# TengdaHan/TemporalAlignNet

Hardware: AMD Instinct MI355X
Metric: video-seq/sec (len=64, E6D6) at 1/2/4/8 MI355X; HTM-Align ROC-AUC parity (higher is better)
Workload: dtype bf16; 1 GPU; E6D6 len=64 bf16 stage-1 (init: multi-positive NCE only) train step (fwd+loss+bwd+AdamW), synthetic HTM-370K-shaped features, N~U[4,16] sentences/video; global_batch=128, per_gpu_batch=128, seq_len=64, parallelism=dp1

## Files before the change

include/tan_hip.h:

```cpp
#ifndef TAN_HIP_H
#define TAN_HIP_H

#ifdef __cplusplus
extern "C" {
#endif

#define TAN_F32 0
#define TAN_BF16 1
#define TAN_ERR_BAD_ARG (-1)

#define TAN_ACT_NONE 0
#define TAN_ACT_QUICKGELU 1
#define TAN_ACT_QUICKGELU_GRAD 2
#define TAN_ACT_RELU 3

int tan_version(void);
int tan_abi_sizeof(int which);

#define TAN_PROF_GEMM_BF16 0
#define TAN_PROF_GEMM_F32 4
#define TAN_PROF_ATTN_FWD 8
#define TAN_PROF_ATTN_BWD 9
#define TAN_PROF_SIMNCE 10
#define TAN_PROF_PANEL 11
// ... 173 lines not shown
    long unit_begin, unit_end;
} tan_adamw_images_desc;
int tan_adamw_step_images(const tan_adamw_images_desc* d, void* stream);
int tan_ema_update(float* target, const float* online, long n, float m, void* target_bf16, void* stream);

int tan_clip_chunk(void);
int tan_clip_sumsq(const float* g, const int* chunk_table, const int* seg_table, int c0, int c1, int s0, int s1, long n,
                   float* partials, void* stream);
int tan_clip_apply(float* g, const int* chunk_table, const int* seg_table, int c0, int c1, int s0, int s1, long n,
                   const float* partials, float clip, float grad_scale, float* norms, void* stream);

typedef struct tan_layer_params {
    const void *w_qkv, *w_out, *w_fc, *w_proj;
    const float *b_qkv, *b_out, *b_fc, *b_proj;
    const float *ln1_g, *ln1_b, *ln2_g, *ln2_b;
    float *g_w_qkv, *g_w_out, *g_w_fc, *g_w_proj;
    float *g_b_qkv, *g_b_out, *g_b_fc, *g_b_proj;
    float *g_ln1_g, *g_ln1_b, *g_ln2_g, *g_ln2_b;
    const void *wt_qkv, *wt_out, *wt_fc, *wt_proj;
    const void *wp_qkv, *wp_out, *wp_fc, *wp_proj;
    const void *wtp_qkv, *wtp_out, *wtp_fc, *wtp_proj;
} tan_layer_params;

typedef struct tan_layer_bufs {
    void *xn1, *qkv, *attn_o, *x_mid, *xn2, *h_pre, *h_act, *x_out;
    float *mean1, *rstd1, *mean2, *rstd2;
    float* lse;
} tan_layer_bufs;

typedef struct tan_encoder_desc {
    int dtype, B, L, C, H, layers;
    const unsigned char* key_padding_mask;
    const void* x0;
    const tan_layer_params* params;
    const tan_layer_bufs* bufs;
    const float *post_g, *post_b;
    float *g_post_g, *g_post_b;
    void* post_out;
    float *post_mean, *post_rstd;
    void *scr_dx, *scr_dx2, *scr_do, *scr_dxn;
    void* scr_dh;
    void* scr_dqkv;
    float* ln_ws;
    float* dw_ws;
    long dw_ws_floats;
    const void* const* d_stage;
    void* d_x0;
    void* const* layer_done;
    int no_save;
    int xn1_ready;
    void* dw_stream; int dw_tail;
    void *scr2_dx, *scr2_dx2, *scr2_dh, *scr2_dqkv;
    float* split_part;
} tan_encoder_desc;
int tan_encoder_fwd(const tan_encoder_desc* e, void* stream);
int tan_encoder_bwd(const tan_encoder_desc* e, void* stream);

int tan_linear_wgrad(const void* dy, const void* x, float* gw, long M, int N, int K, float* ws, long ws_floats, int dtype,
                     void* stream);
int tan_gemm_atb(int n, const void* const* A, const void* const* B, void* const* C, const int* lda, const int* M, const int* N, long K,
                 int out_dtype, int accumulate, int split, void* stream);
int tan_linear_wgrad_group(int n, const void* const* dy, const void* const* x, float* const* gw, const int* N, const int* K,
                           long M, float* ws, long ws_floats, int dtype, void* stream);

typedef struct tan_pack_entry { long src_off, dst_off; int N, K, TN, TK; } tan_pack_entry;
int tan_panel_waves(void);
int tan_pack_weights(const void* src, void* dst, const tan_pack_entry* table, int n, int max_tiles, void* stream);

typedef struct tan_mlp_desc {
    long rows; int C, FF;
    const void* x_mid;
    const float *ln_g, *ln_b;
    const void *pw_fc, *pw_proj;
    const float *b_fc, *b_proj;
    void* xn2; float *mean2, *rstd2;
    void *h_pre, *h_act;
    void* x_out;
    const float *nln_g, *nln_b;
    void* xn_next; float *nmean, *nrstd;
    float eps;
    int variant;
    const void* attn_o; const void* pw_out; const float* b_out; const void* x_in;
} tan_mlp_desc;
int tan_mlp_fwd(const tan_mlp_desc* d, void* stream);

typedef struct tan_mlp_bwd_desc {
    long rows; int C, FF;
    const void* dx;
    const void* h_pre;
    const void* x_mid;
    const float *mean2, *rstd2, *ln_g;
    const void *pwt_proj, *pwt_fc;
    void* dh;
    void* dx2;
    float *g_b_fc, *g_ln_g, *g_ln_b, *g_b_out;
    const void *ln1_dxn, *ln1_x, *ln1_res;
    const float *ln1_mean, *ln1_rstd, *ln1_g;
    float *g_ln1_g, *g_ln1_b, *g_dx_colsum;
    void* dx_out;
    const void* pwt_out;
    void* d_o;
    const void* dqkv;
    const void* pwt_in;
    const void* dstage;
} tan_mlp_bwd_desc;
int tan_mlp_bwd(const tan_mlp_bwd_desc* d, void* stream);
// ... 137 lines not shown
```

temporalalignnet_amd/_lib.py:

```python
from __future__ import annotations

import ctypes as C
import os
import re

HERE = os.path.dirname(os.path.abspath(__file__))
LIB_PATH = os.environ.get("TAN_HIP_LIB") or os.path.join(HERE, "libtan_hip.so")
HEADER = os.path.join(HERE, "..", "include", "tan_hip.h")

TAN_F32, TAN_BF16 = 0, 1
ACT_NONE, ACT_QUICKGELU, ACT_QUICKGELU_GRAD, ACT_RELU = 0, 1, 2, 3


class TanHipError(RuntimeError):
    pass


class GemmDesc(C.Structure):
    _fields_ = [
        ("dtype", C.c_int), ("out_dtype", C.c_int),
        ("M", C.c_int), ("N", C.c_int), ("K", C.c_int),
        ("a_kc", C.c_int), ("b_kc", C.c_int),
        ("A", C.c_void_p), ("lda", C.c_long),
        ("B", C.c_void_p), ("ldb", C.c_long),
# ... 157 lines not shown
        ("pwt_out", C.c_void_p), ("d_o", C.c_void_p),
        ("dqkv", C.c_void_p), ("pwt_in", C.c_void_p), ("dstage", C.c_void_p),
    ]


class EmbedDesc(C.Structure):
    _fields_ = [
        ("a", C.c_void_p), ("a_dtype", C.c_int), ("rows", C.c_long), ("K", C.c_int), ("T", C.c_int), ("C", C.c_int),
        ("pw", C.c_void_p), ("ln_g", C.c_void_p), ("ln_b", C.c_void_p),
        ("a_bf16", C.c_void_p), ("proj", C.c_void_p), ("mean", C.c_void_p), ("rstd", C.c_void_p),
        ("out", C.c_void_p * 2), ("out_grp_rows", C.c_long * 2), ("out_off", C.c_long * 2), ("pos", C.c_void_p * 2),
        ("ln1_g", C.c_void_p * 2), ("ln1_b", C.c_void_p * 2), ("xn1", C.c_void_p * 2), ("mean1", C.c_void_p * 2), ("rstd1", C.c_void_p * 2),
        ("pad_src", C.c_void_p), ("pad_dst", C.c_void_p), ("pad_grp_rows", C.c_long), ("pad_off", C.c_long),
    ]


class EmbedBwdDesc(C.Structure):
    _fields_ = [
        ("rows", C.c_long), ("T", C.c_int), ("C", C.c_int),
        ("d_out", C.c_void_p * 2), ("d_out_grp_rows", C.c_long * 2), ("d_out_off", C.c_long * 2),
        ("proj", C.c_void_p), ("mean", C.c_void_p), ("rstd", C.c_void_p), ("ln_g", C.c_void_p),
        ("d_proj", C.c_void_p), ("g_ln_g", C.c_void_p), ("g_ln_b", C.c_void_p), ("d_pos", C.c_void_p * 2),
    ]


class PosLnBwdUse(C.Structure):
    _fields_ = [("d_pos", C.c_void_p), ("x", C.c_void_p), ("mean", C.c_void_p), ("rstd", C.c_void_p), ("g_table", C.c_void_p), ("n", C.c_int), ("nparts", C.c_int)]


class AttnBlkDesc(C.Structure):
    _fields_ = [
        ("B", C.c_int), ("L", C.c_int), ("C", C.c_int), ("H", C.c_int),
        ("xn1", C.c_void_p), ("x_in", C.c_void_p), ("key_padding_mask", C.c_void_p),
        ("pw_qkv", C.c_void_p), ("pw_out", C.c_void_p), ("b_qkv", C.c_void_p), ("b_out", C.c_void_p),
        ("qkv", C.c_void_p), ("attn_o", C.c_void_p), ("lse", C.c_void_p), ("x_mid", C.c_void_p),
    ]


class EncoderDesc(C.Structure):
    _fields_ = [
        ("dtype", C.c_int), ("B", C.c_int), ("L", C.c_int), ("C", C.c_int), ("H", C.c_int), ("layers", C.c_int),
        ("key_padding_mask", C.c_void_p), ("x0", C.c_void_p),
        ("params", C.POINTER(LayerParams)), ("bufs", C.POINTER(LayerBufs)),
        ("post_g", C.c_void_p), ("post_b", C.c_void_p), ("g_post_g", C.c_void_p), ("g_post_b", C.c_void_p),
        ("post_out", C.c_void_p), ("post_mean", C.c_void_p), ("post_rstd", C.c_void_p),
        ("scr_dx", C.c_void_p), ("scr_dx2", C.c_void_p), ("scr_do", C.c_void_p), ("scr_dxn", C.c_void_p),
        ("scr_dh", C.c_void_p), ("scr_dqkv", C.c_void_p), ("ln_ws", C.c_void_p),
        ("dw_ws", C.c_void_p), ("dw_ws_floats", C.c_long),
        ("d_stage", C.POINTER(C.c_void_p)), ("d_x0", C.c_void_p),
        ("layer_done", C.POINTER(C.c_void_p)),
        ("no_save", C.c_int), ("xn1_ready", C.c_int), ("dw_stream", C.c_void_p), ("dw_tail", C.c_int),
        ("scr2_dx", C.c_void_p), ("scr2_dx2", C.c_void_p), ("scr2_dh", C.c_void_p), ("scr2_dqkv", C.c_void_p),
        ("split_part", C.c_void_p),
    ]


_ROLE_STREAMS = {}


def role_stream(dev, role):
    import torch
    dev = torch.device(dev)
    key = (dev.type, dev.index if dev.index is not None else torch.cuda.current_device(), role)
    st = _ROLE_STREAMS.get(key)
    if st is None:
        for r in ("stack", "loss", "comm", "opt"):
            k = (key[0], key[1], r)
            if k not in _ROLE_STREAMS:
                _ROLE_STREAMS[k] = torch.cuda.Stream(device=torch.device(key[0], key[1]))
        st = _ROLE_STREAMS.setdefault(key, _ROLE_STREAMS.get(key) or torch.cuda.Stream(device=torch.device(key[0], key[1])))
    return st
```

temporalalignnet_amd/csrc/tan_encoder.hip:

```cpp
#include "tan_common.h"
#include <cstdlib>

#ifndef TAN_DW_TARGET_WGS
#define TAN_DW_TARGET_WGS 256
#endif

namespace tal {
int gemm_dw_grouped(int nprob, const void* const* dy, const void* const* x, float* const* parts, const int* Ms, const int* Ns,
                    long rows, int split, int accumulate, hipStream_t st);
int gemm_dw256_grouped(int nprob, const void* const* dy, const void* const* x, float* const* gw, const int* Ms, const int* Ns,
                       long rows, int split, hipStream_t st);
}

using namespace tal;

namespace {

int linear_fwd(int dt, const void* x, const void* w, const float* b, void* y, long M, int N, int K, int act, void* aux,
               const void* residual, void* st) {
    tan_gemm_desc d{};
    d.dtype = dt; d.out_dtype = dt;
    d.M = (int)M; d.N = N; d.K = K;
    d.a_kc = 1; d.b_kc = 1;
    d.A = x; d.lda = K; d.B = w; d.ldb = K; d.C = y; d.ldc = N;
// ... 62 lines not shown
                work += 2.0 * M * it[i].N * (double)it[i].K;
            }
            const int rec = prof_begin((hipStream_t)st, TAN_PROF_GEMM_BF16 + 3, work);
            const int rc = gemm_dw256_grouped(n, dy, x, gw, Ms, Ns, M, s256, (hipStream_t)st);
            prof_end((hipStream_t)st, rec);
            if (rc != -2) return rc;
        }
    }
    if (dt == TAN_BF16 && M % 64 == 0) {
        const void* dy[4]; const void* x[4]; float* parts[4]; int Ms[4], Ns[4];
        double work = 0;
        for (int i = 0; i < n; ++i) {
            dy[i] = it[i].dy; x[i] = it[i].x; parts[i] = it[i].gw; Ms[i] = it[i].N; Ns[i] = it[i].K;
            work += 2.0 * M * it[i].N * (double)it[i].K;
        }
        const int rec = prof_begin((hipStream_t)st, TAN_PROF_GEMM_BF16 + 3, work);
        const int rc = gemm_dw_grouped(n, dy, x, parts, Ms, Ns, M, 1, 1, (hipStream_t)st);
        prof_end((hipStream_t)st, rec);
        if (rc != -2) return rc;
    }
    for (int i = 0; i < n; ++i) CK(linear_bwd_w(dt, it[i].dy, it[i].x, it[i].gw, M, it[i].N, it[i].K, ws, ws_floats, st));
    return 0;
}

}

extern "C" int tan_linear_wgrad_group(int n, const void* const* dy, const void* const* x, float* const* gw, const int* N, const int* K,
                                      long M, float* ws, long ws_floats, int dtype, void* stream) {
    TAN_REQUIRE(n >= 1 && n <= 4 && dy && x && gw && N && K && M > 0);
    DwItem it[4];
    for (int i = 0; i < n; ++i) { TAN_REQUIRE(dy[i] && x[i] && gw[i] && N[i] > 0 && K[i] > 0); it[i] = DwItem{dy[i], x[i], gw[i], N[i], K[i]}; }
    return linear_bwd_w_group(dtype, it, n, M, ws, ws_floats, stream);
}

extern "C" int tan_linear_wgrad(const void* dy, const void* x, float* gw, long M, int N, int K, float* ws, long ws_floats,
                                int dtype, void* stream) {
    TAN_REQUIRE(dy && x && gw && M > 0 && N > 0 && K > 0);
    return linear_bwd_w(dtype, dy, x, gw, M, N, K, ws, ws_floats, stream);
}

static int panel_enabled() {
    static const int on = [] { const char* e = getenv("TAN_PANEL"); return e ? atoi(e) : 1; }();
    return on;
}
static long split_panels() {
    static const long n = [] { const char* e = getenv("TAN_SPLIT_PANELS"); return e ? atol(e) : 48L; }();
    return n;
}
static long split_bwd_panels() {
    static const long n = [] { const char* e = getenv("TAN_SPLIT_BWD_PANELS"); const long v = e ? atol(e) : 24L; return v < split_panels() ? v : split_panels(); }();
    return n;
}

extern "C" int tan_encoder_fwd(const tan_encoder_desc* e, void* st) {
    TAN_REQUIRE(e && e->layers > 0 && e->params && e->bufs && e->x0);
    const int dt = e->dtype, C = e->C, H = e->H;
    const long R = (long)e->B * e->L;
    const void* x_in = e->x0;
    const bool panel_ok = panel_enabled() && dt == TAN_BF16 && C == 512 && R % 64 == 0;
    const bool attn_panel_ok = panel_enabled() && tan_attnblk_supported(e->L, C, H, dt);
    const bool split = panel_ok && e->split_part && R / 64 <= split_panels();
    bool ln1_done = e->xn1_ready != 0;
    for (int i = 0; i < e->layers; ++i) {
        const tan_layer_params& p = e->params[i];
        const tan_layer_bufs& b = e->bufs[i];
        if (!ln1_done) CK(tan_layernorm_fwd(x_in, p.ln1_g, p.ln1_b, b.xn1, b.mean1, b.rstd1, nullptr, 0, R, C, 1e-5f, dt, st));
        ln1_done = false;
        bool out_head = false;
        if (attn_panel_ok && p.wp_qkv && p.wp_out) {
            tan_attnblk_desc ab{};
            ab.B = e->B; ab.L = e->L; ab.C = C; ab.H = H;
            ab.xn1 = b.xn1; ab.x_in = x_in; ab.key_padding_mask = e->key_padding_mask;
            ab.pw_qkv = p.wp_qkv; ab.pw_out = p.wp_out; ab.b_qkv = p.b_qkv; ab.b_out = p.b_out;
            if (!e->no_save) { ab.qkv = b.qkv; ab.attn_o = b.attn_o; ab.lse = b.lse; }
            ab.x_mid = b.x_mid;
            if (split) CK(tan_attnblk_fwd_split(&ab, e->split_part, st));
            else CK(tan_attnblk_fwd(&ab, st));
        } else {
            CK(linear_fwd(dt, b.xn1, p.w_qkv, p.b_qkv, b.qkv, R, 3 * C, C, TAN_ACT_NONE, nullptr, nullptr, st));
            CK(tan_attn_fwd(b.qkv, e->key_padding_mask, b.attn_o, b.lse, e->B, e->L, H, dt, st));
            out_head = panel_ok && !split && p.wp_fc && p.wp_proj && p.wp_out;
            if (!out_head) CK(linear_fwd(dt, b.attn_o, p.w_out, p.b_out, b.x_mid, R, C, C, TAN_ACT_NONE, nullptr, x_in, st));
        }
        if (panel_ok && p.wp_fc && p.wp_proj) {
            tan_mlp_desc m{};
            m.rows = R; m.C = C; m.FF = 4 * C;
            if (out_head) { m.attn_o = b.attn_o; m.pw_out = p.wp_out; m.b_out = p.b_out; m.x_in = x_in; }
            m.x_mid = b.x_mid; m.ln_g = p.ln2_g; m.ln_b = p.ln2_b;
            m.pw_fc = p.wp_fc; m.pw_proj = p.wp_proj; m.b_fc = p.b_fc; m.b_proj = p.b_proj;
            m.x_out = b.x_out;
            if (!e->no_save) { m.xn2 = b.xn2; m.mean2 = b.mean2; m.rstd2 = b.rstd2; m.h_pre = b.h_pre; m.h_act = b.h_act; }
            m.eps = 1e-5f;
            if (i + 1 < e->layers) {
                const tan_layer_params& pn = e->params[i + 1];
                const tan_layer_bufs& bn = e->bufs[i + 1];
                m.nln_g = pn.ln1_g; m.nln_b = pn.ln1_b; m.xn_next = bn.xn1; m.nmean = bn.mean1; m.nrstd = bn.rstd1;
                ln1_done = true;
            } else if (e->post_out) {
                m.nln_g = e->post_g; m.nln_b = e->post_b; m.xn_next = e->post_out; m.nmean = e->post_mean; m.nrstd = e->post_rstd;
                ln1_done = true;
            }
            if (split) CK(tan_mlp_fwd_split(&m, e->split_part, st));
            else CK(tan_mlp_fwd(&m, st));
        } else {
            CK(tan_layernorm_fwd(b.x_mid, p.ln2_g, p.ln2_b, b.xn2, b.mean2, b.rstd2, nullptr, 0, R, C, 1e-5f, dt, st));
            CK(linear_fwd(dt, b.xn2, p.w_fc, p.b_fc, b.h_act, R, 4 * C, C, TAN_ACT_QUICKGELU, b.h_pre, nullptr, st));
            CK(linear_fwd(dt, b.h_act, p.w_proj, p.b_proj, b.x_out, R, C, 4 * C, TAN_ACT_NONE, nullptr, b.x_mid, st));
        }
        x_in = b.x_out;
    }
    if (e->post_out && !ln1_done)
        CK(tan_layernorm_fwd(x_in, e->post_g, e->post_b, e->post_out, e->post_mean, e->post_rstd, nullptr, 0, R, C, 1e-5f, dt, st));
    return 0;
}

extern "C" int tan_encoder_bwd(const tan_encoder_desc* e, void* st) {
    TAN_REQUIRE(e && e->layers > 0 && e->params && e->bufs && e->x0 && e->d_stage && e->d_x0);
    TAN_REQUIRE(e->scr_dx && e->scr_dx2 && e->scr_dh && e->scr_dqkv && e->scr_do && e->scr_dxn && e->ln_ws);
    const int dt = e->dtype, C = e->C, H = e->H, S = e->layers;
    const long R = (long)e->B * e->L;
    const size_t esz = dt == TAN_F32 ? 4 : 2;
    const void* x_last = e->bufs[S - 1].x_out;
    struct { bool on; int layer; const void *dxn, *x, *res; const float *mean, *rstd, *g; float *gg, *gb, *gcol;
             const void *dqkv, *pwt_in, *dstage; } pend{};
    const bool panel_all = panel_enabled() && dt == TAN_BF16 && C == 512 && R % 64 == 0;
    const bool split = panel_all && e->split_part && R / 64 <= split_bwd_panels();
    int tail = e->dw_stream && e->dw_stream != st ? (e->dw_tail > 0 ? e->dw_tail : 0) : 0;
    TAN_REQUIRE(!(tail > 0 && e->layer_done));
    if (tail > S) tail = S;
    if (tail > 16) tail = 16;
    const bool two_sets = e->scr2_dx && e->scr2_dx2 && e->scr2_dh && e->scr2_dqkv;
    if (tail > 1 && !two_sets) tail = 1;
    static thread_local hipEvent_t ev_in = nullptr, ev_done[16] = {};
    if (tail > 0 && !ev_in) {
        if (hipEventCreateWithFlags(&ev_in, hipEventDisableTiming) != hipSuccess) return -3;
        for (int i = 0; i < 16; ++i)
            if (hipEventCreateWithFlags(&ev_done[i], hipEventDisableTiming) != hipSuccess) return -3;
    }
    auto set_b = [&](int i) { return tail > 1 && i < tail && (i & 1); };
    void* dx = set_b(S - 1) ? e->scr2_dx : e->scr_dx;
    if (e->d_stage[S - 1] && panel_all && !split && e->params[S - 1].wtp_fc && e->params[S - 1].wtp_proj) {
        TAN_REQUIRE(e->post_out);
        pend.on = true; pend.layer = -1; pend.dxn = e->d_stage[S - 1]; pend.x = x_last; pend.res = nullptr;
        pend.mean = e->post_mean; pend.rstd = e->post_rstd; pend.g = e->post_g; pend.gg = e->g_post_g; pend.gb = e->g_post_b;
        pend.gcol = e->params[S - 1].g_b_proj;
    } else if (e->d_stage[S - 1]) {
        TAN_REQUIRE(e->post_out);
        CK(tan_layernorm_bwd(e->d_stage[S - 1], x_last, e->post_g, e->post_mean, e->post_rstd, nullptr, dx, e->g_post_g,
                             e->g_post_b, e->params[S - 1].g_b_proj, e->ln_ws, R, C, dt, st));
    } else {
        hipError_t err = hipMemsetAsync(dx, 0, (size_t)R * C * esz, (hipStream_t)st);
        if (err != hipSuccess) return (int)err;
    }
    for (int i = S - 1; i >= 0; --i) {
        const tan_layer_params& p = e->params[i];
        const tan_layer_bufs& b = e->bufs[i];
        const void* x_in = i == 0 ? e->x0 : e->bufs[i - 1].x_out;
        const bool B_ = set_b(i);
        dx = B_ ? e->scr2_dx : e->scr_dx;
        void* const dx2 = B_ ? e->scr2_dx2 : e->scr_dx2;
        void* const scr_dh = B_ ? e->scr2_dh : e->scr_dh;
        void* const scr_dqkv = B_ ? e->scr2_dqkv : e->scr_dqkv;
        if (tail > 1 && i + 2 < tail)
            if (hipStreamWaitEvent((hipStream_t)st, ev_done[i + 2], 0) != hipSuccess) return -3;
        bool do_fused = false;
        if (panel_all && p.wtp_fc && p.wtp_proj) {
// ... 66 lines not shown
```

temporalalignnet_amd/engine.py:

```python
from __future__ import annotations

import collections
import ctypes as C
import os

import numpy as np
import torch

from . import _lib, ops
from .flat_params import _vp
from .workspace import HEADS, WIDTH, _Blocks, _EncRun, _WorkspaceMixin

ChainsResult = collections.namedtuple("ChainsResult", "v_d t_d v_j t_j d_lang out_ev")


class _AlignerFn(torch.autograd.Function):

    @staticmethod
    def forward(ctx, model, video, lang, vmask_u8, tmask_u8, opts, *anchor):
        ctx.set_materialize_grads(False)
        run = model._run_forward(video, lang, vmask_u8, tmask_u8, opts)
        outputs = tuple(run.pop("outputs"))
        ctx.model, ctx.run = model, run
        ctx.lang_requires_grad = lang.requires_grad
# ... 5 lines not shown
        model = ctx.model
        d_lang = model._run_backward(ctx.run, grads, ctx.lang_requires_grad)
        return (None, None, d_lang, None, None, None) + (None,) * ctx.n_anchor


class _AlignerEngine(_WorkspaceMixin):
    def _layer_params(self, prefix, layers):
        f = self._flat
        wbuf = f.shadow if self.compute_dtype == torch.bfloat16 else f.flat
        wt = f.shadow_t if (self.compute_dtype == torch.bfloat16 and self.transposed_dx) else None
        wp = f.shadow_p if (self.compute_dtype == torch.bfloat16 and self.panel_kernels) else None
        wtp = f.shadow_tp if (wt is not None and wp is not None) else None
        sig = (f.flat.data_ptr(), f.grad.data_ptr(), wbuf.data_ptr(), wt.data_ptr() if wt is not None else 0,
               wp.data_ptr() if wp is not None else 0, wtp.data_ptr() if wtp is not None else 0)
        hit = self._lp_cache.get((prefix, layers))
        if hit is not None and hit[0] == sig:
            return hit[1]
        arr = (_lib.LayerParams * layers)()
        m = {"w_qkv": "attn.in_proj_weight", "w_out": "attn.out_proj.weight", "w_fc": "mlp.c_fc.weight",
             "w_proj": "mlp.c_proj.weight"}
        fm = {"b_qkv": "attn.in_proj_bias", "b_out": "attn.out_proj.bias", "b_fc": "mlp.c_fc.bias",
              "b_proj": "mlp.c_proj.bias", "ln1_g": "ln_1.weight", "ln1_b": "ln_1.bias", "ln2_g": "ln_2.weight",
              "ln2_b": "ln_2.bias"}
        for i in range(layers):
            base = f"{prefix}.resblocks.{i}."
            for k, v in m.items():
                setattr(arr[i], k, f.ptr(wbuf, base + v))
                setattr(arr[i], "g_" + k, f.ptr(f.grad, base + v))
                setattr(arr[i], "wt_" + k[2:], f.ptr(wt, base + v) if wt is not None else None)
                setattr(arr[i], "wp_" + k[2:], f.ptr(wp, base + v) if wp is not None else None)
                setattr(arr[i], "wtp_" + k[2:], f.ptr(wtp, base + v) if wtp is not None else None)
            for k, v in fm.items():
                setattr(arr[i], k, f.ptr(f.flat, base + v))
                setattr(arr[i], "g_" + k, f.ptr(f.grad, base + v))
        self._lp_cache[(prefix, layers)] = (sig, arr)
        return arr

    def _enc_desc(self, er: _EncRun, x0, keypad, post_name):
        d = _lib.EncoderDesc()
        d.dtype = ops._dt(x0)
        d.B, d.L, d.C, d.H, d.layers = er.B, er.L, WIDTH, HEADS, er.layers
        d.key_padding_mask = _vp(keypad)
        d.x0 = _vp(x0)
        er.params = self._layer_params(er.prefix, er.layers)
        d.params = er.params
        d.bufs = er.bufs
        d.post_g, d.post_b = _vp(self._f(post_name + ".weight")), _vp(self._f(post_name + ".bias"))
        d.g_post_g, d.g_post_b = _vp(self._g(post_name + ".weight")), _vp(self._g(post_name + ".bias"))
        d.post_out = _vp(er.act["post"])
        d.post_mean, d.post_rstd = _vp(er.stat["post_mean"]), _vp(er.stat["post_rstd"])
        d.split_part = _vp(getattr(er, "split_part", None))
        return d

    def _encoder_fwd(self, er, x0, keypad, post_name, save=False, xn1_ready=False):
        d = self._enc_desc(er, x0, keypad, post_name)
        self._flat.join_images()
        d.no_save = 0 if save else 1
        d.xn1_ready = 1 if xn1_ready else 0
        _lib.check(_lib.lib().tan_encoder_fwd(C.byref(d), ops._stream()), "tan_encoder_fwd")

    def _layer_events(self, prefix, layers):
        cache = self.__dict__.setdefault("_layer_event_cache", {})
        evs = cache.get(prefix)
        if evs is None or len(evs) != layers:
            evs = []
            for _ in range(layers):
                h = C.c_void_p()
                _lib.check(_lib.lib().tan_event_create(C.byref(h)), "tan_event_create")
                evs.append(h.value)
            cache[prefix] = evs
        return evs

    def _encoder_bwd(self, er, x0, keypad, post_name, d_stage, d_x0, dw_stream=None, dw_tail=1):
        cd, dev, R = x0.dtype, x0.device, er.R
        d = self._enc_desc(er, x0, keypad, post_name)
        self._flat.join_images()
        if self._grad_ready_hook is not None:
            evs = self._layer_events(er.prefix, er.layers)
            ev_arr = (C.c_void_p * er.layers)(*evs)
            d.layer_done = ev_arr
        scr = self._take_scratch(R, cd, dev)
        d.scr_dx, d.scr_dx2, d.scr_do, d.scr_dxn = (_vp(scr[k]) for k in ("dx", "dx2", "do", "dxn"))
        d.scr_dh, d.scr_dqkv = _vp(scr["dh"]), _vp(scr["dqkv"])
        d.ln_ws = _vp(scr.ln_ws)
        d.dw_ws, d.dw_ws_floats = _vp(scr.dw_ws), scr.dw_ws.numel()
        arr = (C.c_void_p * er.layers)(*[(t.data_ptr() if t is not None else None) for t in d_stage])
        d.d_stage = arr
        d.d_x0 = _vp(d_x0)
        if dw_stream is not None:
            d.dw_stream, d.dw_tail = C.c_void_p(dw_stream.cuda_stream), dw_tail
            d.scr2_dx, d.scr2_dx2, d.scr2_dh, d.scr2_dqkv = (_vp(scr[k]) for k in ("dx_b", "dx2_b", "dh_b", "dqkv_b"))
        _lib.check(_lib.lib().tan_encoder_bwd(C.byref(d), ops._stream()), "tan_encoder_bwd")

    def _pos_table(self, which):
        return self._f(which) if (which != "temporal_pos_embed" or self.pos_enc == "learned") else self.temporal_pos_embed

    def _pos_ln(self, which, n, start, interpolate_from, cd, keep):
        dev = self._flat.flat.device
        table = self._pos_table(which)
        if interpolate_from:
            src = table[0:interpolate_from].contiguous()
            pos = torch.empty(n, WIDTH, device=dev)
            ops.interp_linear(src, pos, interpolate_from, n, WIDTH)
        else:
            pos = table[start:start + n]
        out = torch.empty(n, WIDTH, device=dev)
        mean, rstd = torch.empty(n, device=dev), torch.empty(n, device=dev)
        ops.layernorm_fwd(pos, self._f("ln_position_init.weight"), self._f("ln_position_init.bias"), out, mean, rstd)
        out_c = out if cd == torch.float32 else ops.cast(out, torch.empty(n, WIDTH, device=dev, dtype=cd))
        saved = {"which": which, "n": n, "start": start, "interp": interpolate_from, "pos": pos, "mean": mean, "rstd": rstd}
        return out_c, saved
# ... 167 lines not shown
                                                 WIDTH, ops._stream()), "tan_pos_ln_bwd")
        cur = torch.cuda.current_stream()
        aux = self._side_stream(dev)
        if aux is not None and aux.cuda_stream == cur.cuda_stream:
            aux = None
        d_lang = None

        def text_side():
            lang_c = sv_t["lang_c"]
            Dt = lang_c.shape[-1]
            ops.gemm(em["dproj_t"], lang_c, self._g("text_pre_proj.weight"), M=WIDTH, N=Dt, K=Mp, a_kc=False, b_kc=False,
                     lda=WIDTH, ldb=Dt, accumulate=True, split_k=max(1, min(16, Mp // 256)))
            if need_d_lang:
                dl = torch.empty(Mp, Dt, dtype=cd, device=dev)
                ops.gemm(em["dproj_t"], self._w("text_pre_proj.weight"), dl, M=Mp, N=Dt, K=WIDTH, a_kc=True, b_kc=False, ldb=Dt)
                return dl.float().view(B, N, Dt)
            return None
        if nprob == 2 and aux is not None:
            aux.wait_stream(cur)
            with torch.cuda.stream(aux):
                d_lang = text_side()
            if d_lang is not None:
                d_lang.record_stream(cur)
        video_c = sv_v["video_c"]
        Dv = video_c.shape[-1]
        ops.gemm(em["dproj_v"], video_c, self._g("video_pre_proj.weight"), M=WIDTH, N=Dv, K=R, a_kc=False, b_kc=False,
                 lda=WIDTH, ldb=Dv, accumulate=True, split_k=max(1, min(32, R // 1024)))
        if nprob == 2:
            if aux is not None:
                cur.wait_stream(aux)
            else:
                d_lang = text_side()
        return d_lang

    def _side_stream(self, dev):
        if not self.overlap_stacks:
            return None
        if self._side is None or self._side.device != dev:
            self._side = _lib.role_stream(dev, "stack")
        return self._side

    def _on_side(self, side, fn):
        if self._issuer is None:
            from concurrent.futures import ThreadPoolExecutor
            self._issuer = ThreadPoolExecutor(max_workers=1, thread_name_prefix="tan-side")
        dev = side.device

        def run():
            torch.cuda.set_device(dev)
            with torch.no_grad(), torch.cuda.stream(side):
                return fn()
        return self._issuer.submit(run)

    def _run_video_stack(self, x0, vmask_u8, B, T, save=False, er=None):
        ready = er is not None
        if er is None:
            er = self._take_ws("video_temporal_encoder", self.num_encoder_layers, B, T, x0.dtype, x0.device)
        self._encoder_fwd(er, x0, vmask_u8, "ln_video_post_enc", save, xn1_ready=ready)
        return er

    def _run_joint_stack(self, x0, text_t, vmask_u8, tmask_u8, B, T, N, save=False, pre=None):
        cd, dev = (x0 if pre is None else pre[1]).dtype, (x0 if pre is None else pre[1]).device
        L = T + N
        if pre is not None:
            er, xj, keypad = pre
            self._encoder_fwd(er, xj, keypad, "ln_joint_post_enc", save, xn1_ready=True)
            er.xj, er.keypad = xj, keypad
            return er
        xj = torch.empty(B * L, WIDTH, dtype=cd, device=dev)
        ops.rows_copy(x0, xj, B, T, WIDTH, T, 0, L, 0)
        ops.rows_copy(text_t, xj, B, N, WIDTH, N, 0, L, T)
        if vmask_u8 is None and tmask_u8 is None:
            keypad = None
        else:
            vm = vmask_u8 if vmask_u8 is not None else torch.zeros(B, T, dtype=torch.uint8, device=dev)
            tm = tmask_u8 if tmask_u8 is not None else torch.zeros(B, N, dtype=torch.uint8, device=dev)
            keypad = torch.cat([vm, tm], dim=1).contiguous()
        er = self._take_ws("joint_temporal_encoder", self.num_decoder_layers, B, L, cd, dev)
        self._encoder_fwd(er, xj, keypad, "ln_joint_post_enc", save)
        er.xj, er.keypad = xj, keypad
        return er

    def _pos_ln_full(self, which):
        f = self._flat
        cache = self.__dict__.setdefault("_pos_ln_cache", {})
        ent = cache.get(which)
        if ent is None or ent["flat"] != f.flat.data_ptr():
            table = self._pos_table(which)
            P, dev = table.shape[0], f.flat.device
            ent = cache[which] = {"flat": f.flat.data_ptr(), "epoch": -1, "out": torch.empty(P, WIDTH, device=dev),
                                  "mean": torch.empty(P, device=dev), "rstd": torch.empty(P, device=dev)}
            if self._pos_ln_refresh not in f.image_hooks:
                f.image_hooks.append(self._pos_ln_refresh)
        if ent["epoch"] != f.shadow_epoch:
            ops.layernorm_fwd(self._pos_table(which).contiguous(), self._f("ln_position_init.weight"), self._f("ln_position_init.bias"),
                              ent["out"], ent["mean"], ent["rstd"])
            ent["epoch"] = f.shadow_epoch
        return ent

    def _pos_ln_refresh(self):
        for which in list(self.__dict__.get("_pos_ln_cache", {})):
            self._pos_ln_full(which)

    def _embed_fused_ok(self, video, lang, itp):
        return (self.compute_dtype == torch.bfloat16 and self.panel_kernels and not itp and video.shape[-1] % 128 == 0
                and lang.shape[-1] % 128 == 0 and video.shape[-1] <= 2048 and lang.shape[-1] <= 2048
                and os.environ.get("TAN_EMBED_FUSED", "1") != "0")

    @staticmethod
    def _feature_operand(x):
        x = x.detach()
        if not x.is_cuda:
            raise _lib.TanHipError("TemporalAligner needs device tensors: the HIP path has no CPU fallback")
        if x.dtype not in (torch.float32, torch.bfloat16):
            x = x.float()
        return x.contiguous()

    def _embed_fused(self, video, lang, vmask_u8, tmask_u8, p_v, p_t, p_j, save):
        f = self._flat
        B, T, Dv = video.shape
        N, Dt = lang.shape[1], lang.shape[2]
        L, R, Mp = T + N, B * T, B * N
        cd, dev = self.compute_dtype, video.device
        video, lang = self._feature_operand(video), self._feature_operand(lang)
        alt = bool(self.__dict__.get("_ws_alternate"))
        ev = self._take_ws("video_temporal_encoder", self.num_encoder_layers, B, T, cd, dev, alternate=alt)
        ej = self._take_ws("joint_temporal_encoder", self.num_decoder_layers, B, L, cd, dev, alternate=alt)
        em = self._take_emb(B, T, N, Dv, Dt, cd, dev)
        pv = self._pos_ln_full("temporal_pos_embed")
        pt = self._pos_ln_full("text_temporal_pos_embed") if self.use_text_pos_enc else None
        f.join_images()
        wp = f.shadow_p
# ... 156 lines not shown
        if which == "video":
            er = self._run_video_stack(fe["x0"], vmask_u8, B, T, False, er=fe["ev"])
            ops.l2norm_fwd_multi([er.stage(self.num_encoder_layers - 1)], vn, inv[:R], R, Cw)
            ops.l2norm_fwd(fe["lang_raw"], tn, inv[R:], Mp, Cw)
        else:
            er = self._run_joint_stack(None, None, vmask_u8, tmask_u8, B, T, N, False, pre=(fe["ej"], fe["xj"], fe["keypad"]))
            last = [er.stage(self.num_decoder_layers - 1)]
            ops.l2norm_fwd_multi(last, vn, inv[:R], R, Cw, T, L, 0)
            ops.l2norm_fwd_multi(last, tn.view(1, Mp, Cw), inv[R:], Mp, Cw, N, L, T)
        out = torch.empty(B, T, N, device=dev)
        ops.gemm(vn[0], tn, out, M=T, N=N, K=Cw, batch=B, sA=T * Cw, sB=N * Cw, sC=T * N)
        self._release_ws(er)
        return out

    def _run_chains(self, video, lang, vmask_u8, tmask_u8, family, after_video_bwd=None, after_joint_bwd=None, pipe=None, mid=None, need_d_lang=False,
                    pre=None):
        self._ensure_flat()
        self._bind_grads()
        f = self._flat
        prev = f.pending if pipe is not None else {}
        B, T, _ = video.shape
        N = lang.shape[1]
        cd, dev = self.compute_dtype, video.device
        Se, Sd, Cw = self.num_encoder_layers, self.num_decoder_layers, WIDTH
        R, Mp, L = B * T, B * N, T + N
        p_v = self._draw(T, None)
        p_t = self._draw(N, None) if self.use_text_pos_enc else 0
        p_j = self._draw(T, None)
        f.sync_shadow_t()
        f.sync_shadow_tp()
        self._ws_alternate = pipe is not None
        try:
            fe = self._embed_fused(video, lang, vmask_u8, tmask_u8, p_v, p_t, p_j, True)
        finally:
            self._ws_alternate = False
        em = fe["em"]
        zero_ev = pipe.get("zero") if pipe is not None else None
        dst_v = torch.empty(Se, R, Cw, dtype=cd, device=dev)
        d_lang_raw = torch.empty(Mp, Cw, dtype=cd, device=dev)
        d_x0 = torch.empty(R, Cw, dtype=cd, device=dev)
        main, side = torch.cuda.current_stream(), self._side_stream(dev)
        serial = bool(getattr(self, "serialize_streams", False))
        if serial:
            side = main
        side.wait_stream(main)
        tail_j, tail_v = 2, 1
        from .workspace import SPLIT_PANELS
        if B * L <= 64 * SPLIT_PANELS:
            tail_j, tail_v = Sd, Se
        aux_j = main if serial else _lib.role_stream(dev, "loss")
        aux_v = main if serial else _lib.role_stream(dev, "opt")
        hook = self._grad_ready_hook
        dw_j, dw_v = (None, None) if hook is not None else (aux_j, aux_v)

        import threading
        joint_terms, joint_ready = [], threading.Event()

        def joint_chain():
            try:
                dst_j = torch.empty(Sd, B * L, Cw, dtype=cd, device=dev)
                d_xj = torch.empty(B * L, Cw, dtype=cd, device=dev)
                if prev.get("joint") is not None:
                    torch.cuda.current_stream().wait_event(prev["joint"])
                if pre is not None:
                    pre["joint"]()
                ej = self._run_joint_stack(None, None, vmask_u8, tmask_u8, B, T, N, True, pre=(fe["ej"], fe["xj"], fe["keypad"]))
                stages = [ej.stage(s) for s in range(Sd)]
                dj = [dst_j[s] for s in range(Sd)]
                if zero_ev is not None:
                    torch.cuda.current_stream().wait_event(zero_ev)
                v_j, t_j = family("joint", stages, (L, 0), stages, (L, T), dj, dj)
                joint_terms.append((v_j, t_j, torch.cuda.current_stream().record_event()))
            finally:
                joint_ready.set()
            self._encoder_bwd(ej, ej.xj, ej.keypad, "ln_joint_post_enc", dj, d_xj, dw_stream=dw_j, dw_tail=tail_j)
            return ej, v_j, t_j, d_xj, (dst_j,)
        fut = self._on_side(side, joint_chain)
        try:
            if prev.get("video") is not None:
                main.wait_event(prev["video"])
            if pre is not None:
                pre["video"]()
            ev = self._run_video_stack(fe["x0"], vmask_u8, B, T, True, er=fe["ev"])
            dv = [dst_v[s] for s in range(Se)]
            if zero_ev is not None:
                main.wait_event(zero_ev)
            v_d, t_d = family("dual", [ev.stage(s) for s in range(Se)], (T, 0), [fe["lang_raw"]], (N, 0), dv, [d_lang_raw])
        except BaseException as main_exc:
            exc = fut.exception()
            if exc is not None and getattr(main_exc, "tan_consequence", False) and not getattr(exc, "tan_consequence", False):
                raise exc
            raise
        self._encoder_bwd(ev, fe["x0"], vmask_u8, "ln_video_post_enc", dv, d_x0, dw_stream=dw_v, dw_tail=tail_v)
        if hook is not None:
            hook("video", self._layer_events(ev.prefix, ev.layers))
        out_ev = {"dw_v": aux_v.record_event() if dw_v is not None else None}
        if after_video_bwd is not None:
            aux_v.wait_stream(main)
            with torch.cuda.stream(aux_v):
                after_video_bwd()
        out_ev["video"] = aux_v.record_event()
        if mid is not None:
            try:
                mid(v_d, t_d, joint_terms, joint_ready)
            except BaseException:
                if fut.done() and fut.exception() is not None:
                    raise fut.exception()
                raise
        ej, v_j, t_j, d_xj, keep = fut.result()
        if hook is not None:
            with torch.cuda.stream(side):
                hook("joint", self._layer_events(ej.prefix, ej.layers))
        out_ev["dw_j"] = aux_j.record_event() if dw_j is not None else None
        if after_joint_bwd is not None:
            aux_j.wait_stream(side)
            with torch.cuda.stream(aux_j):
                after_joint_bwd()
        main.wait_stream(side)
        for t in (d_xj,) + keep:
            t.record_stream(main)
        run = {"em": em, "B": B, "T": T, "N": N, "sv_video": fe["sv_video"], "sv_video_j": fe["sv_video_j"], "sv_text": fe["sv_text"],
               "sv_text_t": fe["sv_text_t"]}
        d_lang = self._embed_bwd_fused(run, d_x0, d_xj, d_lang_raw, need_d_lang)
        out_ev["joint"] = aux_j.record_event()
        if pipe is None:
            main.wait_stream(aux_v)
            main.wait_stream(aux_j)
        self._release_ws(ev)
        self._release_ws(ej)
        self._release_ws(em)
        return ChainsResult(v_d, t_d, v_j, t_j, d_lang, out_ev if pipe is not None else None)

    def _run_backward(self, run, grads, need_d_lang):
        self._bind_grads()
        B, T, N = run["B"], run["T"], run["N"]
        ev, ej = run["ev"], run["ej"]
# ... 175 lines not shown
```

temporalalignnet_amd/tan_model.py:

```python
from __future__ import annotations

import ctypes as C
import os

import numpy as np
import torch
from torch import nn

from . import _lib, ops
from .engine import _AlignerEngine, _AlignerFn
from .flat_params import _ALIGN, _Flat, _vp
from .tfm_model import TemporalEncoder, _LayerNormParams, _LinearParams, get_position_embedding_sine
from .workspace import HEADS, WIDTH


def _local_bert():
    import os
    try:
        from transformers import BertModel
        return BertModel.from_pretrained(os.environ.get("TAN_BERT_PATH", "bert-base-uncased"), local_files_only=True)
    except Exception:
        return None


# ... 7 lines not shown
        self.sim = sim
        self.pos_enc = pos_enc
        self.language_model = language_model
        self.use_text_pos_enc = use_text_pos_enc
        self.return_dual_feature = return_dual_feature
        self.random_pos_start = random_pos_start
        self.use_alignability_head = use_alignability_head
        self.compute_dtype = {"fp32": torch.float32, "bf16": torch.bfloat16, torch.float32: torch.float32,
                              torch.bfloat16: torch.bfloat16}[compute_dtype]
        if num_encoder_layers < 1 or num_decoder_layers < 1:
            raise NotImplementedError("the HIP path needs >= 1 layer per stack (reference edge case tan_model.py:177-179)")

        if language_model == "word2vec":
            from .word2vec_model import Word2VecModel
            self.bert = Word2VecModel(compute_dtype=compute_dtype)
        elif language_model in (None, "none"):
            self.bert = None
        elif language_model == "bert":
            self.bert = _local_bert()
        else:
            raise NotImplementedError(f"language_model={language_model!r}: 'word2vec' (tan_model.py:39-40), 'bert' (:37-38) or None")
        text_embed_dim = {"bert": 768}.get(language_model, 512)

        self.video_temporal_encoder = TemporalEncoder(width=WIDTH, layers=num_encoder_layers, heads=HEADS)
        self.joint_temporal_encoder = TemporalEncoder(width=WIDTH, layers=num_decoder_layers, heads=HEADS)
        self.video_pre_proj = _LinearParams(d_video, WIDTH, bias=False)
        self.text_pre_proj = _LinearParams(text_embed_dim, WIDTH, bias=False)
        self.ln_text_init = _LayerNormParams(WIDTH)
        self.ln_video_init = _LayerNormParams(WIDTH)
        self.ln_position_init = _LayerNormParams(WIDTH)
        self.ln_video_post_enc = _LayerNormParams(WIDTH)
        self.ln_joint_post_enc = _LayerNormParams(WIDTH)
        if pos_enc == "learned":
            self.temporal_pos_embed = nn.Parameter(torch.empty(1024, WIDTH))
            nn.init.normal_(self.temporal_pos_embed, std=0.01)
        elif pos_enc == "sine":
            self.register_buffer("temporal_pos_embed", get_position_embedding_sine(WIDTH, 1024))
        else:
            raise ValueError(pos_enc)
        self.text_temporal_pos_embed = nn.Parameter(torch.empty(1024, WIDTH))
        nn.init.normal_(self.text_temporal_pos_embed, std=0.01)
        self.mlp = _LinearParams(WIDTH, WIDTH)
        if use_alignability_head:
            self.binary_head = _LinearParams(WIDTH, 1)
            nn.init.normal_(self.binary_head.weight, std=0.01)
            nn.init.zeros_(self.binary_head.bias)
        self.initialize_parameters()
        self._flat = _Flat(self, [(n, p) for n, p in self.named_parameters() if not n.startswith("bert.")])
        self._ws_pool, self._ws_lru, self._ws_tick = {}, {}, 0
        import threading
        self._ws_lock = threading.Lock()
        self.overlap_stacks = True
        self.serialize_streams = False
        self._side = None
        self._issuer = None
        self._lp_cache = {}
        self.transposed_dx = True
        self.panel_kernels = os.environ.get("TAN_PANEL", "1") != "0"
        self._grad_ready_hook = None
        self.register_load_state_dict_post_hook(lambda module, incompatible: module.invalidate_shadow())

    def state_dict(self, *args, **kwargs):
        f = self.__dict__.get("_flat")
        if f is not None:
            f.drain()
        return super().state_dict(*args, **kwargs)

    def _drain_pending(self):
        f = self.__dict__.get("_flat")
        if f is not None:
            f.drain()

    def named_parameters(self, *args, **kwargs):
        self._drain_pending()
        return super().named_parameters(*args, **kwargs)

    def invalidate_shadow(self):
        self._drain_pending()
        f = self.__dict__.get("_flat")
        if f is not None:
            f.shadow_version = -1

    def initialize_parameters(self):
        nn.init.normal_(self.video_pre_proj.weight, std=0.01)
        nn.init.normal_(self.text_pre_proj.weight, std=0.01)
        nn.init.normal_(self.mlp.weight, std=0.01)
        nn.init.zeros_(self.mlp.bias)
        w, layers = self.joint_temporal_encoder.width, self.joint_temporal_encoder.layers
        proj_std = (w ** -0.5) * ((2 * layers) ** -0.5)
        attn_std = w ** -0.5
        fc_std = (2 * w) ** -0.5
        for enc in (self.video_temporal_encoder, self.joint_temporal_encoder):
            for blk in enc.resblocks:
                nn.init.normal_(blk.attn.in_proj_weight, std=attn_std)
                nn.init.normal_(blk.attn.out_proj.weight, std=proj_std)
                nn.init.normal_(blk.mlp.c_fc.weight, std=fc_std)
                nn.init.normal_(blk.mlp.c_proj.weight, std=proj_std)

    @property
    def lang_model(self):
        return self.bert

    def _autograd_anchor(self):
        f = self._flat
        for p in f.params:
            if p.requires_grad:
# ... 377 lines not shown
```

Baseline: 31430 video-seq/s.

## Split encoder forward by video groups across two streams

Splits the encoder forward pass into two batches of videos. The first batch runs on the main stream and the second on an auxiliary stream, joined by fork and join events. The aim is to fill the GPU better by overlapping the two halves' kernels, which are serialized per layer. This competes with the joint and video stacks, which already overlap on other streams, and it halves the GEMM M size, which may lower per-kernel efficiency. It only applies when the split-panel path is off, which is not the case for small R.

```diff
diff --git a/include/tan_hip.h b/include/tan_hip.h
--- a/include/tan_hip.h
+++ b/include/tan_hip.h
@@ -249,6 +249,7 @@
     void* dw_stream; int dw_tail;
     void *scr2_dx, *scr2_dx2, *scr2_dh, *scr2_dqkv;
     float* split_part;
+    void* fwd_group_stream; int fwd_group_videos;
 } tan_encoder_desc;
 int tan_encoder_fwd(const tan_encoder_desc* e, void* stream);
 int tan_encoder_bwd(const tan_encoder_desc* e, void* stream);
diff --git a/temporalalignnet_amd/_lib.py b/temporalalignnet_amd/_lib.py
--- a/temporalalignnet_amd/_lib.py
+++ b/temporalalignnet_amd/_lib.py
@@ -233,6 +233,7 @@
         ("no_save", C.c_int), ("xn1_ready", C.c_int), ("dw_stream", C.c_void_p), ("dw_tail", C.c_int),
         ("scr2_dx", C.c_void_p), ("scr2_dx2", C.c_void_p), ("scr2_dh", C.c_void_p), ("scr2_dqkv", C.c_void_p),
         ("split_part", C.c_void_p),
+        ("fwd_group_stream", C.c_void_p), ("fwd_group_videos", C.c_int),
     ]
 
 
diff --git a/temporalalignnet_amd/csrc/tan_encoder.hip b/temporalalignnet_amd/csrc/tan_encoder.hip
--- a/temporalalignnet_amd/csrc/tan_encoder.hip
+++ b/temporalalignnet_amd/csrc/tan_encoder.hip
@@ -138,8 +138,7 @@
     return n;
 }
 
-extern "C" int tan_encoder_fwd(const tan_encoder_desc* e, void* st) {
-    TAN_REQUIRE(e && e->layers > 0 && e->params && e->bufs && e->x0);
+static int encoder_fwd_run(const tan_encoder_desc* e, void* st) {
     const int dt = e->dtype, C = e->C, H = e->H;
     const long R = (long)e->B * e->L;
     const void* x_in = e->x0;
@@ -198,6 +197,71 @@
     if (e->post_out && !ln1_done)
         CK(tan_layernorm_fwd(x_in, e->post_g, e->post_b, e->post_out, e->post_mean, e->post_rstd, nullptr, 0, R, C, 1e-5f, dt, st));
     return 0;
+}
+
+constexpr int FWD_GROUP_MAX_LAYERS = 16;
+
+static void videos_slice(const tan_encoder_desc& e, int v0, int nb, tan_encoder_desc& out, tan_layer_bufs* bufs) {
+    const long r0 = (long)v0 * e.L, C = e.C;
+    const size_t esz = e.dtype == TAN_F32 ? 4 : 2;
+    auto act = [&](auto* p, long width) { return p ? (decltype(p))((char*)p + (size_t)(r0 * width) * esz) : p; };
+    auto vec = [](float* p, long off) { return p ? p + off : p; };
+    out = e;
+    out.B = nb;
+    out.key_padding_mask = e.key_padding_mask ? e.key_padding_mask + r0 : nullptr;
+    out.x0 = act(e.x0, C);
+    out.post_out = act(e.post_out, C);
+    out.post_mean = vec(e.post_mean, r0); out.post_rstd = vec(e.post_rstd, r0);
+    for (int i = 0; i < e.layers; ++i) {
+        const tan_layer_bufs& b = e.bufs[i];
+        tan_layer_bufs& o = bufs[i];
+        o.xn1 = act(b.xn1, C); o.qkv = act(b.qkv, 3 * C); o.attn_o = act(b.attn_o, C); o.x_mid = act(b.x_mid, C); o.xn2 = act(b.xn2, C);
+        o.h_pre = act(b.h_pre, 4 * C); o.h_act = act(b.h_act, 4 * C); o.x_out = act(b.x_out, C);
+        o.mean1 = vec(b.mean1, r0); o.rstd1 = vec(b.rstd1, r0); o.mean2 = vec(b.mean2, r0); o.rstd2 = vec(b.rstd2, r0);
+        o.lse = vec(b.lse, (long)v0 * e.H * e.L);
+    }
+    out.bufs = bufs;
+    out.split_part = nullptr;
+    out.fwd_group_stream = nullptr; out.fwd_group_videos = 0;
+}
+
+static bool fwd_groups_ok(const tan_encoder_desc* e, void* st) {
+    const int g = e->fwd_group_videos;
+    if (!e->fwd_group_stream || e->fwd_group_stream == st || g <= 0 || g >= e->B || e->layers > FWD_GROUP_MAX_LAYERS) return false;
+    const long R = (long)e->B * e->L;
+    const bool panel_ok = panel_enabled() && e->dtype == TAN_BF16 && e->C == 512 && R % 64 == 0;
+    const bool attn_panel_ok = panel_enabled() && tan_attnblk_supported(e->L, e->C, e->H, e->dtype);
+    const bool split = panel_ok && e->split_part && R / 64 <= split_panels();
+    if (!panel_ok || !attn_panel_ok || split) return false;
+    if (((long)g * e->L) % 64 != 0 || ((long)(e->B - g) * e->L) % 64 != 0) return false;
+    for (int i = 0; i < e->layers; ++i) {
+        const tan_layer_params& p = e->params[i];
+        if (!p.wp_qkv || !p.wp_out || !p.wp_fc || !p.wp_proj) return false;
+    }
+    return true;
+}
+
+extern "C" int tan_encoder_fwd(const tan_encoder_desc* e, void* st) {
+    TAN_REQUIRE(e && e->layers > 0 && e->params && e->bufs && e->x0);
+    if (!fwd_groups_ok(e, st)) return encoder_fwd_run(e, st);
+    const hipStream_t s0 = (hipStream_t)st, s1 = (hipStream_t)e->fwd_group_stream;
+    static thread_local hipEvent_t ev_fork = nullptr, ev_join = nullptr;
+    if (!ev_fork) {
+        if (hipEventCreateWithFlags(&ev_fork, hipEventDisableTiming) != hipSuccess) return -3;
+        if (hipEventCreateWithFlags(&ev_join, hipEventDisableTiming) != hipSuccess) return -3;
+    }
+    const int g = e->fwd_group_videos;
+    tan_encoder_desc d0, d1;
+    tan_layer_bufs b0[FWD_GROUP_MAX_LAYERS], b1[FWD_GROUP_MAX_LAYERS];
+    videos_slice(*e, 0, g, d0, b0);
+    videos_slice(*e, g, e->B - g, d1, b1);
+    if (hipEventRecord(ev_fork, s0) != hipSuccess) return -3;
+    if (hipStreamWaitEvent(s1, ev_fork, 0) != hipSuccess) return -3;
+    const int rc0 = encoder_fwd_run(&d0, s0);
+    const int rc1 = encoder_fwd_run(&d1, s1);
+    if (hipEventRecord(ev_join, s1) != hipSuccess) return -3;
+    if (hipStreamWaitEvent(s0, ev_join, 0) != hipSuccess) return -3;
+    return rc0 ? rc0 : rc1;
 }
 
 extern "C" int tan_encoder_bwd(const tan_encoder_desc* e, void* st) {
diff --git a/temporalalignnet_amd/engine.py b/temporalalignnet_amd/engine.py
--- a/temporalalignnet_amd/engine.py
+++ b/temporalalignnet_amd/engine.py
@@ -81,11 +81,21 @@
         d.split_part = _vp(getattr(er, "split_part", None))
         return d
 
-    def _encoder_fwd(self, er, x0, keypad, post_name, save=False, xn1_ready=False):
+    def _fwd_group_videos(self, B, L):
+        mode = getattr(self, "fwd_groups", None)
+        if mode is False or (mode is None and B * L < 128 * 64):
+            return 0
+        gran = 64 // np.gcd(L, 64)
+        return int(B // 2 // gran * gran)
+
+    def _encoder_fwd(self, er, x0, keypad, post_name, save=False, xn1_ready=False, group_stream=None):
         d = self._enc_desc(er, x0, keypad, post_name)
         self._flat.join_images()
         d.no_save = 0 if save else 1
         d.xn1_ready = 1 if xn1_ready else 0
+        g = self._fwd_group_videos(er.B, er.L) if group_stream is not None else 0
+        if g > 0:
+            d.fwd_group_stream, d.fwd_group_videos = C.c_void_p(group_stream.cuda_stream), g
         _lib.check(_lib.lib().tan_encoder_fwd(C.byref(d), ops._stream()), "tan_encoder_fwd")
 
     def _layer_events(self, prefix, layers):
@@ -359,19 +369,19 @@
                 return fn()
         return self._issuer.submit(run)
 
-    def _run_video_stack(self, x0, vmask_u8, B, T, save=False, er=None):
+    def _run_video_stack(self, x0, vmask_u8, B, T, save=False, er=None, group_stream=None):
         ready = er is not None
         if er is None:
             er = self._take_ws("video_temporal_encoder", self.num_encoder_layers, B, T, x0.dtype, x0.device)
-        self._encoder_fwd(er, x0, vmask_u8, "ln_video_post_enc", save, xn1_ready=ready)
+        self._encoder_fwd(er, x0, vmask_u8, "ln_video_post_enc", save, xn1_ready=ready, group_stream=group_stream)
         return er
 
-    def _run_joint_stack(self, x0, text_t, vmask_u8, tmask_u8, B, T, N, save=False, pre=None):
+    def _run_joint_stack(self, x0, text_t, vmask_u8, tmask_u8, B, T, N, save=False, pre=None, group_stream=None):
         cd, dev = (x0 if pre is None else pre[1]).dtype, (x0 if pre is None else pre[1]).device
         L = T + N
         if pre is not None:
             er, xj, keypad = pre
-            self._encoder_fwd(er, xj, keypad, "ln_joint_post_enc", save, xn1_ready=True)
+            self._encoder_fwd(er, xj, keypad, "ln_joint_post_enc", save, xn1_ready=True, group_stream=group_stream)
             er.xj, er.keypad = xj, keypad
             return er
         xj = torch.empty(B * L, WIDTH, dtype=cd, device=dev)
@@ -384,7 +394,7 @@
             tm = tmask_u8 if tmask_u8 is not None else torch.zeros(B, N, dtype=torch.uint8, device=dev)
             keypad = torch.cat([vm, tm], dim=1).contiguous()
         er = self._take_ws("joint_temporal_encoder", self.num_decoder_layers, B, L, cd, dev)
-        self._encoder_fwd(er, xj, keypad, "ln_joint_post_enc", save)
+        self._encoder_fwd(er, xj, keypad, "ln_joint_post_enc", save, group_stream=group_stream)
         er.xj, er.keypad = xj, keypad
         return er
 
@@ -647,6 +657,7 @@
         aux_v = main if serial else _lib.role_stream(dev, "opt")
         hook = self._grad_ready_hook
         dw_j, dw_v = (None, None) if hook is not None else (aux_j, aux_v)
+        grp_j, grp_v = (None, None) if (serial or pre is not None) else (aux_j, aux_v)
 
         import threading
         joint_terms, joint_ready = [], threading.Event()
@@ -659,7 +670,8 @@
                     torch.cuda.current_stream().wait_event(prev["joint"])
                 if pre is not None:
                     pre["joint"]()
-                ej = self._run_joint_stack(None, None, vmask_u8, tmask_u8, B, T, N, True, pre=(fe["ej"], fe["xj"], fe["keypad"]))
+                ej = self._run_joint_stack(None, None, vmask_u8, tmask_u8, B, T, N, True, pre=(fe["ej"], fe["xj"], fe["keypad"]),
+                                           group_stream=grp_j)
                 stages = [ej.stage(s) for s in range(Sd)]
                 dj = [dst_j[s] for s in range(Sd)]
                 if zero_ev is not None:
@@ -676,7 +688,7 @@
                 main.wait_event(prev["video"])
             if pre is not None:
                 pre["video"]()
-            ev = self._run_video_stack(fe["x0"], vmask_u8, B, T, True, er=fe["ev"])
+            ev = self._run_video_stack(fe["x0"], vmask_u8, B, T, True, er=fe["ev"], group_stream=grp_v)
             dv = [dst_v[s] for s in range(Se)]
             if zero_ev is not None:
                 main.wait_event(zero_ev)
diff --git a/temporalalignnet_amd/tan_model.py b/temporalalignnet_amd/tan_model.py
--- a/temporalalignnet_amd/tan_model.py
+++ b/temporalalignnet_amd/tan_model.py
@@ -83,6 +83,7 @@
         self._ws_lock = threading.Lock()
         self.overlap_stacks = True
         self.serialize_streams = False
+        self.fwd_groups = None
         self._side = None
         self._issuer = None
         self._lp_cache = {}
```

After: 31800 video-seq/s, median of 6. 1.01x the previous value.
